# ShenhanQian/SpeechDrivesTemplates

Measured on AMD Instinct MI355X. Metric: training clips/sec (64-frame, 137-kpt) voice2pose_sdt_bp, higher is better.
Workload: dtype f32 (Conv2d forward / input gradient: each fp32 operand split exactly into three bf16 numbers, six bf16 MFMA products per fp32 product, fp32 accumulation -- products exact to 2^-23; everything else fp32 arithmetic)

## Files before the change

__graft_entry__.py:

```python
import os
import subprocess
import sys

REPO = os.path.dirname(os.path.abspath(__file__))
CSRC = os.path.join(REPO, "speechdrivestemplates_amd", "csrc")
LIBDIR = os.path.join(REPO, "speechdrivestemplates_amd", "lib")
LIB = os.path.join(LIBDIR, "libsdt_hip.so")
SOURCES = ["conv.hip", "convsk.hip", "convbf.hip", "norm.hip", "misc.hip", "l0.hip", "chain1d.hip", "render.hip", "speaker_stats.hip",
           "code_pca.hip", "code_axes.hip", "code_clusters.hip", "fgd.hip", "jpeg.hip", "gif.hip", "clip_builder.hip", "optim_guard.hip",
           "tensor_hist.hip", "reg_loss.hip", "clip_metrics.hip", "long_demo.hip"]
HIPCC = os.environ.get("HIPCC", "/opt/rocm/bin/hipcc")
FLAGS = ["--offload-arch=gfx950", "-O3", "-std=c++17", "-fPIC", "-munsafe-fp-atomics", "-Wno-unused-result", "-Wno-unused-value"]


def _stale(out, deps):
    if not os.path.exists(out):
        return True
    t = os.path.getmtime(out)
    return any(os.path.getmtime(d) > t for d in deps)


TUNING_LIB = os.path.join(LIBDIR, "libsdt_hip_tuning.so")


def _headers():
    return sorted(os.path.join(CSRC, f) for f in os.listdir(CSRC) if f.endswith(".h")) + [os.path.join(REPO, "include", "sdt_hip.h")]


def _start_compiles(prefix, extra, force):
    objs, procs = [], []
    for src in SOURCES:
        s = os.path.join(CSRC, src)
        o = os.path.join(LIBDIR, prefix + src.replace(".hip", ".o"))
        objs.append(o)
        if force or _stale(o, [s] + _headers()):
            procs.append((src, subprocess.Popen([HIPCC] + FLAGS + extra + ["-c", s, "-o", o])))
    return objs, procs


def _finish(lib, objs, procs, force):
    for src, p in procs:
        if p.wait() != 0:
            raise RuntimeError("hipcc failed on %s (%s)" % (src, os.path.basename(lib)))
    if force or procs or _stale(lib, objs):
        subprocess.check_call([HIPCC, "--offload-arch=gfx950", "-shared", "-fPIC", "-o", lib] + objs)


def build_tuning(force=False):
    os.makedirs(LIBDIR, exist_ok=True)
    objs, procs = _start_compiles("tuning_", ["-DSDT_TUNING"], force)
    _finish(TUNING_LIB, objs, procs, force)
    return TUNING_LIB


def build(force=False):
    os.makedirs(LIBDIR, exist_ok=True)
    objs, procs = _start_compiles("", [], force)
    tobjs, tprocs = _start_compiles("tuning_", ["-DSDT_TUNING"], force)
    _finish(LIB, objs, procs, force)
    _finish(TUNING_LIB, tobjs, tprocs, force)
    if REPO not in sys.path:
        sys.path.insert(0, REPO)
    import speechdrivestemplates_amd
    from speechdrivestemplates_amd import _lib
    _lib.load()


def make_pipeline(cfg_name, n_clips, batch_global=None, state=None, log_interval=10 ** 9, sys_opts=None):
    if REPO not in sys.path:
        sys.path.insert(0, REPO)
    from speechdrivestemplates_amd.config import get_cfg_defaults
    from speechdrivestemplates_amd.core.datasets import gesture_dataset as gd
    from speechdrivestemplates_amd.core.pipelines import get_pipeline
    cfg = get_cfg_defaults()
    cfg.merge_from_file(os.path.join(REPO, "configs", cfg_name + ".yaml"))
    opts = ["DATASET.NAME", "SyntheticGestureDataset", "DATASET.SYNTHETIC_CLIPS", n_clips, "SYS.LOG_INTERVAL", log_interval]
    if batch_global is not None:
        opts += ["TRAIN.BATCH_SIZE", batch_global]
    for k, v in (sys_opts or {}).items():
        opts += ["SYS." + k, v]
    cfg.merge_from_list(opts)
    cfg.freeze()
    pipe = get_pipeline(cfg.PIPELINE_TYPE)(cfg)
    pipe.num_train_samples = n_clips
    pipe.train_dataset = gd.SyntheticGestureDataset(cfg=cfg, num_clips=n_clips)
    kw = {}
    if cfg.PIPELINE_TYPE == "Voice2Pose" and cfg.VOICE2POSE.GENERATOR.CLIP_CODE.EXTERNAL_CODE:
        import numpy as np
        import torch
        kw["external_codes"] = torch.from_numpy(np.random.Generator(np.random.PCG64(9)).standard_normal(
            (n_clips, cfg.VOICE2POSE.GENERATOR.CLIP_CODE.DIMENSION)).astype("float32"))
    pipe.setup_model(cfg, state_dict=None if state is None else {"module." + k: v for k, v in state.items()}, **kw)
    pipe.setup_optimizer()
# ... 43 lines not shown
```

include/sdt_hip.h:

```cpp
#ifndef SDT_HIP_H
#define SDT_HIP_H

#include <stdint.h>

#ifdef __cplusplus
extern "C" {
#endif

#define SDT_MAX_TAPS 20

enum sdt_status { SDT_OK = 0, SDT_ERR_ARG = -1, SDT_ERR_LAUNCH = -2, SDT_ERR_UNSUPPORTED = -3 };
enum sdt_dtype { SDT_F32 = 0, SDT_BF16 = 1 };

const char* sdt_last_error(void);
int sdt_abi_version(void);

typedef struct sdt_conv_geom {
    int32_t B, Hi, Wi, Cin;
    int32_t Ho, Wo;
    int32_t Hy, Wy, Cout;
    int32_t sy, sx;
    int32_t osy, osx, ooy, oox;
    int32_t ntaps, Tw;
    int32_t dy[SDT_MAX_TAPS], dx[SDT_MAX_TAPS], wt[SDT_MAX_TAPS];
// ... 98 lines not shown
                         int64_t rows, int C, float eps, float slope, void* stream);
int sdt_colnorm_bwd_f32(const float* dz, const float* y, float* dy, double* sums, const float* mean,
                        const float* rstd, const float* gamma, const float* beta, float* dgamma,
                        float* dbeta, int G, int64_t R, int C, float slope, int stats_ready, void* stream);
int sdt_colnorm_bwd_t(const void* dz, int dz_dtype, const void* y, int y_dtype, void* dy, int dy_dtype, double* sums, const float* mean,
                      const float* rstd, const float* gamma, const float* beta, float* dgamma,
                      float* dbeta, int G, int64_t R, int C, float slope, int stats_ready, void* stream);

int sdt_l0_block_fwd_f32(const float* mel, const float* w, float* z, double* mom, float* mean, float* rstd,
                         const float* gamma, const float* beta, float* running_mean, float* running_var,
                         int64_t* num_batches_tracked, int B, int H, int W, int groups, float eps, float momentum,
                         float slope, void* stream);
int sdt_l0_block_bwd_f32(const float* dz, const float* mel, const float* w, const float* mean, const float* rstd,
                         const float* gamma, const float* beta, const double* mom, double* sums, float* dw, float* dgamma,
                         float* dbeta, int B, int H, int W, int groups, float slope, void* stream);
int sdt_l0_block_fwd_t(const float* mel, const float* w, void* z, int z_dtype, double* mom, float* mean, float* rstd,
                       const float* gamma, const float* beta, float* running_mean, float* running_var,
                       int64_t* num_batches_tracked, int B, int H, int W, int groups, float eps, float momentum,
                       float slope, void* stream);
int sdt_l0_block_bwd_t(const void* dz, int dz_dtype, const float* mel, const float* w, const float* mean, const float* rstd,
                       const float* gamma, const float* beta, const double* mom, double* sums, float* dw, float* dgamma,
                       float* dbeta, int B, int H, int W, int groups, float slope, void* stream);

int sdt_rownorm_fwd_f32(const float* y, float* z, float* mean, float* rstd, int64_t rows, int C,
                        float eps, float slope, void* stream);
int sdt_rownorm_bwd_f32(const float* dz, const float* y, const float* mean, const float* rstd, float* dy,
                        int64_t rows, int C, float slope, void* stream);
int sdt_rownorm_slabs_fwd_f32(const float* partial, int nslab, float* y, float* z, float* mean, float* rstd,
                              int64_t rows, int C, float eps, float slope, void* stream);

int sdt_resize_concat_fwd_f32(const float* x, const float* table, const int64_t* idx, float* out,
                              int B, int H, int W, int C, int T, int D, void* stream);
int sdt_resize_concat_bwd_f32(const float* dout, const int64_t* idx, float* dx, float* dtable,
                              int B, int H, int W, int C, int T, int D, void* stream);

int sdt_upsample_add_fwd_f32(const float* prev, const float* skip, float* out, int B, int Ti, int To, int C, void* stream);
int sdt_upsample_add_bwd_f32(const float* dout, float* dprev, int B, int Ti, int To, int C, void* stream);

enum { SDT_CHAIN_PLAIN = 0, SDT_CHAIN_NORM = 1, SDT_CHAIN_UPADD = 2 };
typedef struct sdt_chain1d_layer {
    int32_t Ti, To, Cin, k, stride, pad;
    int32_t in_mode;
    int32_t src_a, src_b;
    int32_t reserved;
    const float* w;
    const float* wt;
    float* y;
    float* x;
    float* dy;
    float* dx;
} sdt_chain1d_layer;
int sdt_chain1d_supported(const sdt_chain1d_layer* layers, int nlayers, int B);
int sdt_chain1d_fwd_f32(const sdt_chain1d_layer* layers, int nlayers, const float* x0, float* zout, int B, float slope, float eps,
                        int math, void* counters, void* err, void* stream);
int sdt_chain1d_bwd_f32(const sdt_chain1d_layer* layers, int nlayers, const float* gz, int B, float slope, float eps, int need_dx0,
                        int math, void* counters, void* err, void* stream);

int sdt_l1_loss_fwd_f32(const float* pred, const float* gt, int64_t n, float lambda, double* partial, float* loss, void* stream);
int sdt_l1_loss_bwd_f32(const float* pred, const float* gt, const float* gout, int64_t n, float lambda, float* dpred, void* stream);
int sdt_reg_loss_fwd_f32(const float* pred, const float* gt, const float* score, const float* chan_w, int B, int T, int C,
                         double lambda_reg, double lambda_vel, float min_conf, double* partial, int64_t* counts, float* losses,
                         double* denom, void* stream);
int sdt_reg_loss_bwd_f32(const float* pred, const float* gt, const float* score, const float* chan_w, const float* gout_reg,
                         const float* gout_vel, const double* denom, int B, int T, int C, double lambda_reg, double lambda_vel,
                         float min_conf, float* dpred, void* stream);
int sdt_mse_const_fwd_f32(const float* scores, int64_t n, float target, float lambda, float* loss, void* stream);
int sdt_mse_const_bwd_f32(const float* scores, const float* gout, int64_t n, float target, float lambda, float* dscores, void* stream);

int sdt_code_kl_fwd_f32(const float* table, const int64_t* idx, int N, int B, int D, float lambda,
                        float* code_out, float* loss, int32_t* valid, void* stream);
int sdt_code_kl_bwd_f32(const float* code, const int32_t* valid, const float* gout, const int64_t* idx,
                        int N, int B, int D, float lambda, float* dtable, void* stream);

int sdt_final_metrics_f64(const float* pred, const float* gt, const double* mean, const double* std,
                          const double* scale, int hierarchical, int B, int T, int K,
                          double* final_pred, double* final_gt, double* work, double* metrics, void* stream);

int sdt_adam_step_f32(float* p, const float* g, float* m, float* v, int64_t n, const float* lr_dev, float beta1,
                      float beta2, float eps, float weight_decay, float grad_scale, void* state_dev, void* stream);

int sdt_stft_frames_f32(const float* audio, float* hops, int B, int L, int nhops, void* stream);
int sdt_mel_fb_f32(const float* spec, const float* fb, const int32_t* bin_lo, const int32_t* bin_hi, float* mel, int B, int F,
                   int nfreq, int nmel, void* stream);

int sdt_rows_scatter_add_f32(const float* src, const int64_t* idx, float* dst, int N, int B, int D, void* stream);

int sdt_time_diff_fwd_f32(const float* x, float* y, int B, int T, int C, void* stream);
int sdt_time_diff_bwd_f32(const float* dy, float* dx, int B, int T, int C, void* stream);

int sdt_clip_poses_prepare_f32(const float* raw, const int64_t* idx, const float* mean, const float* std, float* poses,
                               float* score, int N, int Tstore, int B, int T, int hierarchical, void* stream);
int sdt_rows_gather_f32(const float* src, const int64_t* idx, float* dst, int N, int B, int64_t n_cols, void* stream);

typedef struct sdt_render_instance {
    int64_t pose;
    double off_x, off_y;
    double scale;
    int32_t shift_x;
    int32_t clip_x0, clip_x1;
    int32_t reserved;
} sdt_render_instance;

int64_t sdt_render_workspace_bytes(int n_images, int n_inst, int K);
int sdt_render_edges(int K);
int sdt_render_prepare_f64(const double* poses, int64_t n_poses, int K, const sdt_render_instance* inst, int n_images, int n_inst,
                           int H, int W, void* workspace, int64_t workspace_bytes, int32_t* skipped, void* stream);
int sdt_render_skeleton_u8(const void* workspace, int64_t workspace_bytes, int n_images, int n_inst, int K, int H, int W,
                           uint8_t* out, int64_t out_bytes, void* stream);

int64_t sdt_speaker_stats_state_bytes(int num_chunks, int num_frames);
int sdt_speaker_stats_accumulate(int pass, int elem_bytes, const void* poses, int64_t poses_elems, int64_t chunk_pitch, int num_chunks,
                                 int num_frames, int window, int64_t first_row, int64_t rows_per_chunk, const double* mean137, void* state,
                                 int64_t state_bytes, void* stream);
int sdt_speaker_stats_finalize(int pass, const void* state, int64_t state_bytes, int num_chunks, int num_frames, double* out137,
                               double* out242, double* counts, int64_t* first_bad_row, int32_t* flags, void* stream);

int64_t sdt_code_pca_workspace_bytes(int64_t n_rows, int dim);
int sdt_code_pca_moments(const float* x, int64_t n_rows, int dim, void* workspace, int64_t workspace_bytes, double* mean, double* cov,
                         int64_t* first_bad_row, void* stream);
int sdt_code_pca_eigh(const double* cov, int dim, int max_sweeps, double rel_tol, double* evals, double* comps, double* info, int32_t* err,
                      void* stream);
int sdt_code_pca_project(const float* x, int64_t n_rows, int dim, const double* mean, const double* comps, double* X, void* workspace,
                         int64_t workspace_bytes, double* limits, void* stream);
int sdt_code_pca_raster(const double* X, int64_t n_rows, const double* axis_limits, const uint8_t* table, int table_len, int H, int W,
                        int margin, int marker_px, uint32_t* counts, int64_t counts_elems, uint8_t* out, int64_t out_bytes, void* stream);

int sdt_code_axes_eigh(const double* cov, int dim, int max_sweeps, double rel_tol, double* evals, double* comps, double* info, int32_t* err,
                       void* stream);
int sdt_code_axes_project(const float* x, int64_t n_rows, int dim, const double* mean, const double* comps, double* P, void* stream);
int64_t sdt_code_axes_quantiles_workspace_bytes(int64_t n_rows, int dim, int n_ranks);
int sdt_code_axes_quantiles(const double* P, int64_t n_rows, int dim, const int64_t* ranks, int n_ranks, double* out, void* workspace,
                            int64_t workspace_bytes, void* stream);
int64_t sdt_code_axes_nearest_workspace_bytes(int64_t n_rows, int dim, int64_t n_queries);
int sdt_code_axes_nearest(const float* x, int64_t n_rows, int dim, const double* queries, int64_t n_queries, int64_t* index, double* dist2,
                          int64_t* first_bad_query, void* workspace, int64_t workspace_bytes, void* stream);

int64_t sdt_code_clusters_seed_workspace_bytes(int64_t n_rows, int dim);
int sdt_code_clusters_seed_update(const float* x, int64_t n_rows, int dim, const int64_t* seeds, int j, int first, double* m, void* workspace,
                                  int64_t workspace_bytes, void* stream);
int sdt_code_clusters_seed_pick(const double* m, int64_t n_rows, int mode, double u, int64_t* seeds, int j, double* info, void* workspace,
                                int64_t workspace_bytes, void* stream);
int sdt_code_clusters_assign(const float* x, int64_t n_rows, int dim, const double* centers, int k, int32_t* labels, int first, int64_t* changed,
                             void* stream);
int64_t sdt_code_clusters_update_workspace_bytes(int64_t n_rows, int dim, int k);
int sdt_code_clusters_update(const float* x, int64_t n_rows, int dim, const int32_t* labels, int k, double* centers, int32_t* counts,
                             void* workspace, int64_t workspace_bytes, void* stream);
int64_t sdt_code_clusters_final_workspace_bytes(int64_t n_rows, int dim, int k);
int sdt_code_clusters_final(const float* x, int64_t n_rows, int dim, const double* centers, int k, int32_t* labels, double* centers_out,
                            int32_t* counts, double* within_ss, double* inertia, int64_t* code_index, double* code_dist2, int32_t* order,
                            void* workspace, int64_t workspace_bytes, void* stream);

int64_t sdt_fgd_state_bytes(int dim);
int sdt_fgd_accumulate(const float* x0, int d0, const float* x1, int d1, int64_t rows, void* state, int64_t state_bytes,
                       int64_t rows_seen_base, void* stream);
int sdt_fgd_finalize(const void* const* states_a, const void* const* states_b, int num_states, int dim, int dim_used, int max_sweeps,
                     double rel_tol, double* out, int32_t* err, void* stream);

#define SDT_JPEG_TABLE_WORDS 672
#define SDT_JPEG_ERR_STAGE 1
#define SDT_JPEG_ERR_RANGE 2
int64_t sdt_jpeg_workspace_bytes(int n, int H, int W);
int64_t sdt_jpeg_intervals(int n, int H, int W);
int sdt_jpeg_measure(const uint8_t* frames, int64_t frames_bytes, int n, int H, int W, const uint32_t* tables, void* workspace,
                     int64_t workspace_bytes, int64_t* offsets, int64_t offsets_elems, int32_t* err, void* stream);
int sdt_jpeg_pack(const void* workspace, int64_t workspace_bytes, int n, int H, int W, const uint32_t* tables, const int64_t* offsets,
                  int64_t offsets_elems, uint8_t* out, int64_t out_bytes, int32_t* err, void* stream);
// ... 71 lines not shown
```

speechdrivestemplates_amd/_lib.py:

```python
import ctypes as C
import os

_HERE = os.path.dirname(os.path.abspath(__file__))
LIB_PATH = os.environ.get("SDT_HIP_LIB") or os.path.join(_HERE, "lib", "libsdt_hip.so")
MAX_TAPS = 20
ABI_VERSION = 5


class ConvGeom(C.Structure):
    _fields_ = [(n, C.c_int32) for n in
                ("B", "Hi", "Wi", "Cin", "Ho", "Wo", "Hy", "Wy", "Cout", "sy", "sx", "osy", "osx", "ooy", "oox",
                 "ntaps", "Tw")] + [("dy", C.c_int32 * MAX_TAPS), ("dx", C.c_int32 * MAX_TAPS), ("wt", C.c_int32 * MAX_TAPS)]


class NormBwd(C.Structure):
    _fields_ = [("y", C.c_void_p), ("mean", C.c_void_p), ("rstd", C.c_void_p), ("gamma", C.c_void_p), ("beta", C.c_void_p),
                ("sums", C.c_void_p), ("slope", C.c_float), ("groups", C.c_int32)]


class WtDesc(C.Structure):
    _fields_ = [("w", C.c_void_p), ("wt", C.c_void_p), ("w16", C.c_void_p), ("wt16", C.c_void_p), ("cout", C.c_int32), ("taps", C.c_int32),
                ("cin", C.c_int32), ("tile_begin", C.c_int32), ("planes", C.c_int32), ("reserved", C.c_int32)]


class ChainLayer(C.Structure):
    _fields_ = [("Ti", C.c_int32), ("To", C.c_int32), ("Cin", C.c_int32), ("k", C.c_int32), ("stride", C.c_int32), ("pad", C.c_int32),
                ("in_mode", C.c_int32), ("src_a", C.c_int32), ("src_b", C.c_int32), ("reserved", C.c_int32),
                ("w", C.c_void_p), ("wt", C.c_void_p), ("y", C.c_void_p), ("x", C.c_void_p), ("dy", C.c_void_p), ("dx", C.c_void_p)]


CHAIN_PLAIN, CHAIN_NORM, CHAIN_UPADD = 0, 1, 2
_p, _i, _i64, _f = C.c_void_p, C.c_int, C.c_int64, C.c_float
_G = C.POINTER(ConvGeom)

SIGNATURES = {
    "sdt_conv_taps_f32": [_p, _p, _p, _p, _G, _p],
    "sdt_conv_dw_f32": [_p, _p, _p, _G, _p],
    "sdt_conv_dw_det_f32": [_p, _p, _p, _G, _p, _i64, _p],
    "sdt_conv_taps_splitk_hint": [_G],
    "sdt_conv_taps_splitk_f32": [_p, _p, _p, _p, _G, _i, _p, _p],
    "sdt_splitk_reduce_f32": [_p, _p, _p, _i64, _i, _i, _p],
    "sdt_conv_taps_variant": [_G],
    "sdt_conv1d_small_used": [_G, _i, _i],
    "sdt_conv_dw_variant": [_G],
    "sdt_weight_transpose_f32": [_p, _p, _i, _i, _i, _p],
    "sdt_weight_transpose_batched_f32": [_p, _i, _i, _p],
    "sdt_set_conv_math": [_i],
    "sdt_col_sum_f32": [_p, _p, _i64, _i, _p],
    "sdt_colnorm_fwd_f32": [_p, _p, _p, _p, _p, _p, _p, _p, _p, _p, _i, _i64, _i, _f, _f, _f, _i, _p],
    "sdt_colnorm_fwd_t": [_p, _i, _p, _i, _p, _p, _p, _p, _p, _p, _p, _p, _i, _i64, _i, _f, _f, _f, _i, _p],
    "sdt_conv_taps_stats_supported": [_G, _i],
    "sdt_conv_taps_stats_f32": [_p, _p, _p, _p, _G, _p, _i, _p],
    "sdt_colnorm_eval_f32": [_p, _p, _p, _p, _p, _p, _i64, _i, _f, _f, _p],
    "sdt_colnorm_bwd_f32": [_p, _p, _p, _p, _p, _p, _p, _p, _p, _p, _i, _i64, _i, _f, _i, _p],
    "sdt_colnorm_bwd_t": [_p, _i, _p, _i, _p, _i, _p, _p, _p, _p, _p, _p, _p, _i, _i64, _i, _f, _i, _p],
    "sdt_conv_taps_multi_f32": [_p, _p, _p, _G, _i, _i, _p, C.POINTER(NormBwd), _p],
    "sdt_l0_block_fwd_f32": [_p, _p, _p, _p, _p, _p, _p, _p, _p, _p, _p, _i, _i, _i, _i, _f, _f, _f, _p],
    "sdt_l0_block_bwd_f32": [_p, _p, _p, _p, _p, _p, _p, _p, _p, _p, _p, _p, _i, _i, _i, _i, _f, _p],
    "sdt_l0_block_fwd_t": [_p, _p, _p, _i, _p, _p, _p, _p, _p, _p, _p, _p, _i, _i, _i, _i, _f, _f, _f, _p],
    "sdt_l0_block_bwd_t": [_p, _i, _p, _p, _p, _p, _p, _p, _p, _p, _p, _p, _p, _i, _i, _i, _i, _f, _p],
    "sdt_rownorm_fwd_f32": [_p, _p, _p, _p, _i64, _i, _f, _f, _p],
    "sdt_rownorm_bwd_f32": [_p, _p, _p, _p, _p, _i64, _i, _f, _p],
    "sdt_rownorm_slabs_fwd_f32": [_p, _i, _p, _p, _p, _p, _i64, _i, _f, _f, _p],
    "sdt_resize_concat_fwd_f32": [_p, _p, _p, _p, _i, _i, _i, _i, _i, _i, _p],
    "sdt_resize_concat_bwd_f32": [_p, _p, _p, _p, _i, _i, _i, _i, _i, _i, _p],
    "sdt_upsample_add_fwd_f32": [_p, _p, _p, _i, _i, _i, _i, _p],
    "sdt_conv_dw_group_plan": [C.POINTER(_G), _i, _p, C.POINTER(C.c_int64)],
    "sdt_conv_dw_group_f32": [C.POINTER(C.c_void_p), C.POINTER(C.c_void_p), C.POINTER(C.c_void_p), _i, _p, _p, _p, _p],
    "sdt_chain1d_supported": [C.POINTER(ChainLayer), _i, _i],
    "sdt_chain1d_fwd_f32": [C.POINTER(ChainLayer), _i, _p, _p, _i, _f, _f, _i, _p, _p, _p],
    "sdt_chain1d_bwd_f32": [C.POINTER(ChainLayer), _i, _p, _i, _f, _f, _i, _i, _p, _p, _p],
    "sdt_upsample_add_bwd_f32": [_p, _p, _i, _i, _i, _i, _p],
    "sdt_l1_loss_fwd_f32": [_p, _p, _i64, _f, _p, _p, _p],
    "sdt_l1_loss_bwd_f32": [_p, _p, _p, _i64, _f, _p, _p],
    "sdt_reg_loss_fwd_f32": [_p, _p, _p, _p, _i, _i, _i, C.c_double, C.c_double, _f, _p, _p, _p, _p, _p],
    "sdt_reg_loss_bwd_f32": [_p, _p, _p, _p, _p, _p, _p, _i, _i, _i, C.c_double, C.c_double, _f, _p, _p],
    "sdt_mse_const_fwd_f32": [_p, _i64, _f, _f, _p, _p],
    "sdt_mse_const_bwd_f32": [_p, _p, _i64, _f, _f, _p, _p],
    "sdt_code_kl_fwd_f32": [_p, _p, _i, _i, _i, _f, _p, _p, _p, _p],
    "sdt_code_kl_bwd_f32": [_p, _p, _p, _p, _i, _i, _i, _f, _p, _p],
    "sdt_final_metrics_f64": [_p, _p, _p, _p, _p, _i, _i, _i, _i, _p, _p, _p, _p, _p],
    "sdt_adam_step_f32": [_p, _p, _p, _p, _i64, _p, _f, _f, _f, _f, _f, _p, _p],
    "sdt_stft_frames_f32": [_p, _p, _i, _i, _i, _p],
    "sdt_mel_fb_f32": [_p, _p, _p, _p, _p, _i, _i, _i, _i, _p],
    "sdt_rows_scatter_add_f32": [_p, _p, _p, _i, _i, _i, _p],
    "sdt_time_diff_fwd_f32": [_p, _p, _i, _i, _i, _p],
    "sdt_time_diff_bwd_f32": [_p, _p, _i, _i, _i, _p],
    "sdt_clip_poses_prepare_f32": [_p, _p, _p, _p, _p, _p, _i, _i, _i, _i, _i, _p],
    "sdt_rows_gather_f32": [_p, _p, _p, _i, _i, _i64, _p],
    "sdt_convsk_supported": [_G, _i],
    "sdt_convsk_grid": [],
    "sdt_convsk_set_wg_per_cu": [_i],
    "sdt_convsk_set_f32_split": [_i],
    "sdt_convsk_set_reserved_slots": [_i],
    "sdt_convsk_plan_build": [_G, _i, _i, _i, _p, _i64],
    "sdt_convsk_dw_supported": [_G],
    "sdt_convsk_dw_plan_build": [_G, _p, _i64],
    "sdt_convsk_dw_f32": [_p, _p, _p, _p, _p, _p, _i64, _i64, _p],
    "sdt_convsk_f32": [_p, _p, _p, _p, _p, _p, _p, C.c_uint, _p, C.POINTER(NormBwd), _i64, _i64, _i64, _p],
    "sdt_convsk_bf16": [_p, _p, _p, _p, _p, _p, _p, C.c_uint, _p, C.POINTER(NormBwd), _i64, _i64, _i64, _p],
    "sdt_convsk_f32_w3": [_p, _p, _p, _p, _p, _p, _p, C.c_uint, _p, C.POINTER(NormBwd), _i64, _i64, _i64, _p],
    "sdt_convsk_supported_t": [_G, _i, _i],
    "sdt_convsk_plan_build_t": [_G, _i, _i, _i, _i, _i, _p, _i64],
    "sdt_convsk_dw_supported_t": [_G, _i],
    "sdt_convsk_dw_plan_build_t": [_G, _i, _p, _i64],
    "sdt_convsk_dw_bf16": [_p, _p, _p, _p, _p, _p, _i64, _i64, _p],
    "sdt_convsk_set_spin_limit": [C.c_uint],
    "sdt_convsk_set_k_order": [_i],
    "sdt_convsk_set_dw_wide_tiles": [_i],
    "sdt_render_workspace_bytes": [_i, _i, _i],
    "sdt_render_edges": [_i],
    "sdt_render_prepare_f64": [_p, _i64, _i, _p, _i, _i, _i, _i, _p, _i64, _p, _p],
    "sdt_render_skeleton_u8": [_p, _i64, _i, _i, _i, _i, _i, _p, _i64, _p],
    "sdt_speaker_stats_state_bytes": [_i, _i],
    "sdt_speaker_stats_accumulate": [_i, _i, _p, _i64, _i64, _i, _i, _i, _i64, _i64, _p, _p, _i64, _p],
    "sdt_speaker_stats_finalize": [_i, _p, _i64, _i, _i, _p, _p, _p, _p, _p, _p],
    "sdt_code_pca_workspace_bytes": [_i64, _i],
    "sdt_code_pca_moments": [_p, _i64, _i, _p, _i64, _p, _p, _p, _p],
    "sdt_code_pca_eigh": [_p, _i, _i, C.c_double, _p, _p, _p, _p, _p],
    "sdt_code_pca_project": [_p, _i64, _i, _p, _p, _p, _p, _i64, _p, _p],
    "sdt_code_pca_raster": [_p, _i64, _p, _p, _i, _i, _i, _i, _i, _p, _i64, _p, _i64, _p],
    "sdt_code_axes_eigh": [_p, _i, _i, C.c_double, _p, _p, _p, _p, _p],
    "sdt_code_axes_project": [_p, _i64, _i, _p, _p, _p, _p],
    "sdt_code_axes_quantiles_workspace_bytes": [_i64, _i, _i],
    "sdt_code_axes_quantiles": [_p, _i64, _i, _p, _i, _p, _p, _i64, _p],
    "sdt_code_axes_nearest_workspace_bytes": [_i64, _i, _i64],
    "sdt_code_axes_nearest": [_p, _i64, _i, _p, _i64, _p, _p, _p, _p, _i64, _p],
    "sdt_code_clusters_seed_workspace_bytes": [_i64, _i],
    "sdt_code_clusters_seed_update": [_p, _i64, _i, _p, _i, _i, _p, _p, _i64, _p],
    "sdt_code_clusters_seed_pick": [_p, _i64, _i, C.c_double, _p, _i, _p, _p, _i64, _p],
    "sdt_code_clusters_assign": [_p, _i64, _i, _p, _i, _p, _i, _p, _p],
    "sdt_code_clusters_update_workspace_bytes": [_i64, _i, _i],
    "sdt_code_clusters_update": [_p, _i64, _i, _p, _i, _p, _p, _p, _i64, _p],
    "sdt_code_clusters_final_workspace_bytes": [_i64, _i, _i],
    "sdt_code_clusters_final": [_p, _i64, _i, _p, _i, _p, _p, _p, _p, _p, _p, _p, _p, _p, _i64, _p],
    "sdt_fgd_state_bytes": [_i],
    "sdt_fgd_accumulate": [_p, _i, _p, _i, _i64, _p, _i64, _i64, _p],
    "sdt_fgd_finalize": [C.POINTER(C.c_void_p), C.POINTER(C.c_void_p), _i, _i, _i, _i, C.c_double, _p, _p, _p],
    "sdt_jpeg_workspace_bytes": [_i, _i, _i],
    "sdt_jpeg_intervals": [_i, _i, _i],
    "sdt_jpeg_measure": [_p, _i64, _i, _i, _i, _p, _p, _i64, _p, _i64, _p, _p],
    "sdt_jpeg_pack": [_p, _i64, _i, _i, _i, _p, _p, _i64, _p, _i64, _p, _p],
    "sdt_gif_workspace_bytes": [_i, _i, _i],
    "sdt_gif_quantise": [_p, _i64, _i, _i, _i, _i, _i, _p, _i64, _p, _i64, _p, _p, _i64, _p],
    "sdt_gif_measure": [_p, _i64, _i, _i, _i, _p, _i64, _p, _i64, _p, _p],
    "sdt_gif_pack": [_p, _i64, _i, _i, _i, _p, _i64, _p, _i64, _p, _p],
    "sdt_clip_workspace_bytes": [_i64],
    "sdt_clip_frame_flags": [_i, _p, _p, _i64, _p, _p, _p, _p],
    "sdt_clip_scan": [_p, _p, _i64, _p, _p, _p],
    "sdt_clip_shoulder_means": [_p, _p, _i64, _i, _p, _p],
    "sdt_clip_window_candidates": [_i64, _i, _i, _i],
    "sdt_clip_windows": [_p, _i64, _i, _i, _i, _p, _i64, _p, _i64, _p, _p],
    "sdt_clip_gather_poses": [_i, _p, _i64, _p, _i64, _i, C.c_double, _i, _p, _i64, _p],
    "sdt_clip_pcm_to_mono_f32": [_i, _p, _i64, _i, _i64, _p, _i64, _p],
    "sdt_clip_resample_lds_bytes": [_i, _i, _i],
    "sdt_clip_resample_f32": [_p, _i64, _p, _i, _i, _i, _i64, _p, _i64, _p],
    "sdt_clip_gather_audio": [_p, _i64, _p, _p, _i64, _i64, _p, _i64, _p, _p],
    "sdt_grad_sumsq_partials": [],
    "sdt_optim_guard_pass_elems": [_i],
    "sdt_grad_sumsq_f64": [_p, _i64, _p, _p],
    "sdt_optim_guard_prep": [C.POINTER(C.c_void_p), _i, _f, C.c_double, _i, _p, _p],
    "sdt_adam_step_guarded_f32": [_p, _p, _p, _p, _i64, _p, _f, _f, _f, _f, _p, _p, _f, _p, _p],
    "sdt_tensor_hist_threads": [],
    "sdt_tensor_hist_chunk": [],
    "sdt_tensor_hist_buckets": [],
    "sdt_tensor_hist_max_segments": [],
    "sdt_tensor_hist_plan": [_p, _i, _i64, _p, _p, _i64, _p],
# ... 99 lines not shown
```

speechdrivestemplates_amd/mel.py:

```python
import math

import torch
from torch import nn

from . import ops


def htk_filterbank(n_freqs, f_min, f_max, n_mels, sample_rate):
    freqs = torch.linspace(0, sample_rate // 2, n_freqs)
    mel_lo = 2595.0 * math.log10(1.0 + f_min / 700.0)
    mel_hi = 2595.0 * math.log10(1.0 + f_max / 700.0)
    edges = 700.0 * (10 ** (torch.linspace(mel_lo, mel_hi, n_mels + 2) / 2595.0) - 1.0)
    width = edges[1:] - edges[:-1]
    dist = edges.unsqueeze(0) - freqs.unsqueeze(1)
    rising = -dist[:, :-2] / width[:-1]
    falling = dist[:, 2:] / width[1:]
    return torch.minimum(rising, falling).clamp_min(0.0)


class _Window(nn.Module):
    def __init__(self, win_length):
        super().__init__()
        self.register_buffer('window', torch.hann_window(win_length, periodic=True))


class _MelScale(nn.Module):
    def __init__(self, n_freqs, f_min, f_max, n_mels, sample_rate):
        super().__init__()
        self.register_buffer('fb', htk_filterbank(n_freqs, f_min, f_max, n_mels, sample_rate))


class MelSpectrogram(nn.Module):
    def __init__(self, sample_rate=16000, n_fft=512, win_length=400, hop_length=160, f_min=55, f_max=7500.0, n_mels=80):
        super().__init__()
        if (n_fft, win_length, hop_length) != (ops.N_FFT, ops.WIN, ops.HOP):
            raise NotImplementedError('the STFT kernel path is specialised to n_fft=512 / win=400 / hop=160')
        self.spectrogram = _Window(win_length)
        self.mel_scale = _MelScale(n_fft // 2 + 1, float(f_min), float(f_max), n_mels, sample_rate)
        self._basis = None
        self._basis_key = None
        self._bins = None
        self._bins_key = None

    def _dft_basis(self):
        w = self.spectrogram.window
        key = (w.data_ptr(), w._version, w.device)
        if self._basis is None or self._basis_key != key:
            self._basis = ops.dft_basis(w).to(w.device)
            self._basis_key = key
        return self._basis

    def _fb_bins(self):
        fb = self.mel_scale.fb
        key = (fb.data_ptr(), fb._version, fb.device)
        if self._bins is None or self._bins_key != key:
            self._bins = ops.fb_bin_ranges(fb)
            self._bins_key = key
        return self._bins

    @torch.no_grad()
    def forward(self, waveform):
        return ops.mel_spectrogram(waveform, self._dft_basis(), self.mel_scale.fb, self._fb_bins())
```

speechdrivestemplates_amd/ops.py:

```python
import functools
import math
import os

import torch

from . import _lib
from ._lib import ConvGeom, check

LEAKY_SLOPE = 0.2
BN_EPS, BN_MOMENTUM = 1e-5, 0.1


def out_size(n, k, s, p):
    return (n + 2 * p - k) // s + 1


def _geom(**kw):
    g = ConvGeom()
    taps = kw.pop("taps")
    for k, v in kw.items():
        setattr(g, k, int(v))
    g.ntaps = len(taps)
    assert 0 < g.ntaps <= _lib.MAX_TAPS, "kernel has too many taps (%d)" % g.ntaps
    for i, (dy, dx, wt) in enumerate(taps):
# ... 1668 lines not shown
class TimeDiffFn(torch.autograd.Function):

    @staticmethod
    def forward(ctx, x):
        _req_cuda(x)
        x = x.contiguous()
        B, T, C = x.shape
        y = torch.empty((B, T - 1, C), device=x.device, dtype=torch.float32)
        check(_lib.load().sdt_time_diff_fwd_f32(_p(x), _p(y), B, T, C, _stream()))
        ctx.dims = (B, T, C)
        return y

    @staticmethod
    def backward(ctx, g):
        B, T, C = ctx.dims
        g = g.contiguous()
        dx = torch.empty((B, T, C), device=g.device, dtype=torch.float32)
        check(_lib.load().sdt_time_diff_bwd_f32(_p(g), _p(dx), B, T, C, _stream()))
        return dx


def clip_poses_prepare(raw_store, idx, mean, std, num_frames, hierarchical):
    _req_cuda(raw_store, idx, mean, std)
    assert raw_store.dim() == 4 and raw_store.shape[2:] == (3, 137) and raw_store.is_contiguous() and raw_store.dtype == torch.float32
    assert idx.dtype == torch.int64 and mean.numel() == 242 and std.numel() == 242
    N, Tstore = raw_store.shape[:2]
    B = idx.numel()
    poses = torch.empty((B, num_frames, 2, 121), device=raw_store.device, dtype=torch.float32)
    score = torch.empty_like(poses)
    idx, mean, std = idx.contiguous(), mean.contiguous(), std.contiguous()
    check(_lib.load().sdt_clip_poses_prepare_f32(_p(raw_store), _p(idx), _p(mean), _p(std),
                                                 _p(poses), _p(score), N, Tstore, B, num_frames, int(bool(hierarchical)), _stream()))
    return poses, score


def rows_gather(src, idx):
    _req_cuda(src, idx)
    assert src.dim() == 2 and src.is_contiguous() and src.dtype == torch.float32 and idx.dtype == torch.int64
    dst = torch.empty((idx.numel(), src.shape[1]), device=src.device, dtype=torch.float32)
    idx = idx.contiguous()
    check(_lib.load().sdt_rows_gather_f32(_p(src), _p(idx), _p(dst), src.shape[0], idx.numel(), src.shape[1], _stream()))
    return dst


def final_metrics(pred, gt, mean, std, scale, hierarchical, want_final=True):
    _req_cuda(pred, gt, mean, std, scale)
    B, T, _, K = pred.shape
    pred, gt = pred.contiguous(), gt.contiguous()
    dev = pred.device
    fp = torch.empty((B, T, 2, K), device=dev, dtype=torch.float64) if want_final else None
    fg = torch.empty((B, T, 2, K), device=dev, dtype=torch.float64) if want_final else None
    work = _ARENA.take(3 * B * T + 4, dev)
    metrics = torch.empty(2, device=dev, dtype=torch.float64)
    mean, std, scale = mean.contiguous(), std.contiguous(), scale.contiguous()
    check(_lib.load().sdt_final_metrics_f64(_p(pred), _p(gt), _p(mean), _p(std), _p(scale),
                                            1 if hierarchical else 0, B, T, K, _p(fp), _p(fg), _p(work), _p(metrics), _stream()))
    return fp, fg, metrics


N_FFT, WIN, HOP, N_FREQ = 512, 400, 160, 257


def dft_basis(window):
    w = window.detach().double().cpu()
    k = torch.arange(WIN, dtype=torch.float64)
    f = torch.arange(N_FREQ, dtype=torch.float64)
    ang = 2.0 * math.pi * torch.outer(f, k + (N_FFT - WIN) // 2) / N_FFT
    basis = torch.zeros(2 * N_FREQ, 3 * HOP, dtype=torch.float64)
    basis[0::2, :WIN] = torch.cos(ang) * w
    basis[1::2, :WIN] = -torch.sin(ang) * w
    return basis.float().reshape(2 * N_FREQ, 3, HOP).contiguous()


def fb_bin_ranges(fb):
    nz = (fb.detach().cpu() != 0)
    n_freq = nz.shape[0]
    idx = torch.arange(n_freq).unsqueeze(1)
    lo = torch.where(nz, idx, torch.full_like(idx, n_freq)).min(0).values
    hi = torch.where(nz, idx + 1, torch.zeros_like(idx)).max(0).values
    lo = torch.minimum(lo, hi)
    return lo.to(torch.int32).to(fb.device), hi.to(torch.int32).to(fb.device)


def mel_spectrogram(audio, basis, fb, bins=None):
    _req_cuda(audio, basis, fb)
    lo, hi = bins if bins is not None else fb_bin_ranges(fb)
    lib = _lib.load()
    audio = audio.contiguous()
    B, L = audio.shape
    F = 1 + L // HOP
    nh = F + 2
    st = _stream()
    hops = torch.empty((B, nh, HOP), device=audio.device, dtype=torch.float32)
    check(lib.sdt_stft_frames_f32(_p(audio), _p(hops), B, L, nh, st))
    g = _geom(B=B, Hi=1, Wi=nh, Cin=HOP, Ho=1, Wo=F, Hy=1, Wy=F, Cout=2 * N_FREQ, sy=1, sx=1, osy=1, osx=1, ooy=0, oox=0,
              Tw=3, taps=[(0, 0, 0), (0, 1, 1), (0, 2, 2)])
    spec = torch.empty((B, F, 2 * N_FREQ), device=audio.device, dtype=torch.float32)
    math = _CONV_MATH_NOW[0]
    if math != 0:
        check(lib.sdt_set_conv_math(0))
    try:
        check(lib.sdt_conv_taps_f32(_p(hops), _p(basis), None, _p(spec), g, st))
    finally:
        if math != 0:
            check(lib.sdt_set_conv_math(math))
    nmel = fb.shape[1]
    mel = torch.empty((B, nmel, F), device=audio.device, dtype=torch.float32)
    fb = fb.contiguous()
    check(lib.sdt_mel_fb_f32(_p(spec), _p(fb), _p(lo), _p(hi), _p(mel), B, F, N_FREQ, nmel, st))
    return mel


def adam_step(p, g, m, v, lr_dev, state_dev, beta1=0.9, beta2=0.999, eps=1e-8, weight_decay=0.0, grad_scale=1.0):
    _req_cuda(p, g, m, v, lr_dev, state_dev)
    check(_lib.load().sdt_adam_step_f32(_p(p), _p(g), _p(m), _p(v), p.numel(), _p(lr_dev), beta1, beta2, eps, weight_decay,
                                        grad_scale, _p(state_dev), _stream()))


GUARD_WORDS = 4


def grad_sumsq_partials():
    return int(_lib.load().sdt_grad_sumsq_partials())


def optim_guard_pass_elems(which):
    return int(_lib.load().sdt_optim_guard_pass_elems({'sumsq': 0, 'adam': 1}[which]))


def grad_sumsq(g, partial):
    _req_cuda(g, partial)
    if g.dtype != torch.float32 or partial.dtype != torch.float64 or partial.numel() < grad_sumsq_partials():
        raise ValueError('grad_sumsq: g must be fp32 and partial %d float64 elements' % grad_sumsq_partials())
    check(_lib.load().sdt_grad_sumsq_f64(_p(g), g.numel(), _p(partial), _stream()))
    return partial


def optim_guard_prep(partials, guard, grad_scale=1.0, max_norm=0.0, skip_nonfinite=False):
    _req_cuda(guard, *partials)
    if not 1 <= len(partials) <= 4:
        raise ValueError('a step group has 1 to 4 buffers, got %d' % len(partials))
    if guard.dtype != torch.int64 or guard.numel() < GUARD_WORDS:
        raise ValueError('the guard record is %d int64 words' % GUARD_WORDS)
    import ctypes as C
    arr = (C.c_void_p * len(partials))(*[_p(t) for t in partials])
    check(_lib.load().sdt_optim_guard_prep(arr, len(partials), grad_scale, float(max_norm), int(bool(skip_nonfinite)), _p(guard), _stream()))


def adam_step_guarded(p, g, m, v, lr_dev, state_dev, guard, beta1=0.9, beta2=0.999, eps=1e-8, weight_decay=0.0, ema=None, ema_decay=0.0):
    _req_cuda(p, g, m, v, lr_dev, state_dev, guard)
    if ema is not None:
        _req_cuda(ema)
        if ema.numel() != p.numel() or ema.dtype != torch.float32:
            raise ValueError('the EMA buffer must match the parameter buffer')
    check(_lib.load().sdt_adam_step_guarded_f32(_p(p), _p(g), _p(m), _p(v), p.numel(), _p(lr_dev), beta1, beta2, eps, weight_decay,
                                                _p(guard), _p(ema), ema_decay, _p(state_dev), _stream()))


def _check_sizes(status):
    if status == -3:
        raise ValueError('libsdt_hip: %s' % _lib.load().sdt_last_error().decode())
    check(status)


def tensor_hist_constants():
    lib = _lib.load()
    return {k: int(getattr(lib, 'sdt_tensor_hist_' + k)()) for k in ('threads', 'chunk', 'buckets', 'max_segments')}


def tensor_hist_plan(offsets, sizes, n):
    import ctypes as C
    lib = _lib.load()
    S = len(offsets)
    if len(sizes) != S:
        raise ValueError('tensor_hist_plan: %d offsets but %d sizes' % (S, len(sizes)))
    segs = torch.tensor([[int(o), int(s)] for o, s in zip(offsets, sizes)], dtype=torch.int64).reshape(S, 2)
    n_chunks = C.c_int64(0)
    _check_sizes(lib.sdt_tensor_hist_plan(_p(segs) if S else None, S, int(n), None, None, 0, C.addressof(n_chunks)))
    seg_plan = torch.zeros((S, 3), dtype=torch.int64)
    chunk_plan = torch.zeros((max(1, n_chunks.value), 2), dtype=torch.int64)
    _check_sizes(lib.sdt_tensor_hist_plan(_p(segs), S, int(n), _p(seg_plan), _p(chunk_plan), n_chunks.value, C.addressof(n_chunks)))
    return seg_plan, chunk_plan[:n_chunks.value]


def tensor_hist(flat, seg_plan, chunk_plan, edges, scale, counts, tallies, stats, partials):
    _req_cuda(flat, seg_plan, chunk_plan, edges, counts, tallies, stats, partials)
    S, nc = seg_plan.shape[0], chunk_plan.shape[0]
    if flat.dtype != torch.float32 or not flat.is_contiguous():
        raise ValueError('tensor_hist: flat must be a contiguous fp32 buffer')
    if counts.dtype != torch.int64 or tallies.dtype != torch.int64 or stats.dtype != torch.float64 or edges.dtype != torch.float64 \
            or counts.numel() < S * (edges.numel() - 1) or tallies.numel() < 3 * S or stats.numel() < 4 * S or partials.numel() < 4 * nc \
# ... 5 lines not shown
```

Before: 5696.

## Fuse STFT power into compact-bin MFMA kernel for mel spectrogram

Adds a dedicated STFT kernel that computes only the frequency bins the mel filterbank actually uses, over a compacted, zero-trimmed DFT basis, and squares real/imag inside the kernel to emit power directly. A new filterbank kernel then reads that compact power tensor. This replaces the generic full-spectrum conv plus separate filterbank pass, cutting wasted MACs on dead bins and the full complex spectrum round trip. The compacted basis is cached per module, and it adds code paths that must match the old numerics.

```diff
diff --git a/__graft_entry__.py b/__graft_entry__.py
--- a/__graft_entry__.py
+++ b/__graft_entry__.py
@@ -8,7 +8,7 @@
 LIB = os.path.join(LIBDIR, "libsdt_hip.so")
 SOURCES = ["conv.hip", "convsk.hip", "convbf.hip", "norm.hip", "misc.hip", "l0.hip", "chain1d.hip", "render.hip", "speaker_stats.hip",
            "code_pca.hip", "code_axes.hip", "code_clusters.hip", "fgd.hip", "jpeg.hip", "gif.hip", "clip_builder.hip", "optim_guard.hip",
-           "tensor_hist.hip", "reg_loss.hip", "clip_metrics.hip", "long_demo.hip"]
+           "tensor_hist.hip", "reg_loss.hip", "clip_metrics.hip", "long_demo.hip", "mel.hip"]
 HIPCC = os.environ.get("HIPCC", "/opt/rocm/bin/hipcc")
 FLAGS = ["--offload-arch=gfx950", "-O3", "-std=c++17", "-fPIC", "-munsafe-fp-atomics", "-Wno-unused-result", "-Wno-unused-value"]
 
diff --git a/include/sdt_hip.h b/include/sdt_hip.h
--- a/include/sdt_hip.h
+++ b/include/sdt_hip.h
@@ -204,6 +204,12 @@
 int sdt_stft_frames_f32(const float* audio, float* hops, int B, int L, int nhops, void* stream);
 int sdt_mel_fb_f32(const float* spec, const float* fb, const int32_t* bin_lo, const int32_t* bin_hi, float* mel, int B, int F,
                    int nfreq, int nmel, void* stream);
+int sdt_mel_compact_map(int k0, int k1, int32_t* src_row, int cap);
+int sdt_mel_basis_compact_f32(const float* basis, int nfreq, int k0, int k1, float* out, void* stream);
+int sdt_stft_power_f32(const float* hops, const float* basis_c, float* power, int B, int nhops, int F, int nbins_live, int ncols,
+                       int klen, void* stream);
+int sdt_mel_fb_power_f32(const float* power, const float* fb, const int32_t* bin_lo, const int32_t* bin_hi, float* mel, int B, int F,
+                         int k0, int nbins_live, int nmel, void* stream);
 
 int sdt_rows_scatter_add_f32(const float* src, const int64_t* idx, float* dst, int N, int B, int D, void* stream);
 
diff --git a/speechdrivestemplates_amd/_lib.py b/speechdrivestemplates_amd/_lib.py
--- a/speechdrivestemplates_amd/_lib.py
+++ b/speechdrivestemplates_amd/_lib.py
@@ -83,6 +83,10 @@
     "sdt_adam_step_f32": [_p, _p, _p, _p, _i64, _p, _f, _f, _f, _f, _f, _p, _p],
     "sdt_stft_frames_f32": [_p, _p, _i, _i, _i, _p],
     "sdt_mel_fb_f32": [_p, _p, _p, _p, _p, _i, _i, _i, _i, _p],
+    "sdt_mel_compact_map": [_i, _i, _p, _i],
+    "sdt_mel_basis_compact_f32": [_p, _i, _i, _i, _p, _p],
+    "sdt_stft_power_f32": [_p, _p, _p, _i, _i, _i, _i, _i, _i, _p],
+    "sdt_mel_fb_power_f32": [_p, _p, _p, _p, _p, _i, _i, _i, _i, _i, _p],
     "sdt_rows_scatter_add_f32": [_p, _p, _p, _i, _i, _i, _p],
     "sdt_time_diff_fwd_f32": [_p, _p, _i, _i, _i, _p],
     "sdt_time_diff_bwd_f32": [_p, _p, _i, _i, _i, _p],
diff --git a/speechdrivestemplates_amd/csrc/mel.hip b/speechdrivestemplates_amd/csrc/mel.hip
--- /dev/null
+++ b/speechdrivestemplates_amd/csrc/mel.hip
@@ -0,0 +1,216 @@
+#include "common.h"
+
+#define STP_BM 64
+#define STP_BINS 32
+#define STP_BK 32
+#define STP_LDP 36
+#define STP_K 480
+#define STP_OOB 0x80000000u
+
+__host__ __device__ static inline int mel_compact_src(int n, int k0, int k1) {
+    const int bin = k0 + (n / (2 * STP_BINS)) * STP_BINS + (n % STP_BINS);
+    return bin < k1 ? 2 * bin + ((n / STP_BINS) & 1) : -1;
+}
+static inline int mel_compact_cols(int k0, int k1) { return cdiv(k1 - k0, STP_BINS) * 2 * STP_BINS; }
+
+__global__ __launch_bounds__(256) void mel_basis_compact_kernel(const float* __restrict__ basis, float* __restrict__ out, int k0, int k1,
+                                                                int ncols) {
+    const int total = ncols * STP_K;
+    for (int i = blockIdx.x * 256 + threadIdx.x; i < total; i += gridDim.x * 256) {
+        const int n = i / STP_K, k = i - n * STP_K;
+        const int src = mel_compact_src(n, k0, k1);
+        out[i] = src >= 0 ? basis[(size_t)src * STP_K + k] : 0.f;
+    }
+}
+
+__global__ __launch_bounds__(128) void stft_power_kernel(const float* __restrict__ X, const float* __restrict__ W, float* __restrict__ P,
+                                                         const int B, const int nh, const int F, const int nbl, const int ncols,
+                                                         const int nsteps) {
+    __shared__ __attribute__((aligned(16))) float sA[STP_BM * STP_LDP];
+    __shared__ __attribute__((aligned(16))) float sB[2 * STP_BINS * STP_LDP];
+    const int tid = threadIdx.x, lane = tid & 63, wave = tid >> 6;
+    const int M = B * F;
+    const int nmb = (M + STP_BM - 1) / STP_BM, nnb = ncols / (2 * STP_BINS);
+    const int lin = xcd_remap(blockIdx.x, nmb * nnb);
+    const int m0 = (lin / nnb) * STP_BM, nt = lin % nnb;
+
+    const int kv = tid & 7, r0 = tid >> 3;
+    const __amdgpu_buffer_rsrc_t rsX = __builtin_amdgcn_make_buffer_rsrc((void*)X, 0, (int)((unsigned)B * nh * 160u * 4u), 0x00020000);
+    const __amdgpu_buffer_rsrc_t rsW = __builtin_amdgcn_make_buffer_rsrc((void*)W, 0, (int)((unsigned)ncols * STP_K * 4u), 0x00020000);
+    unsigned aoff[4], boff[4];
+#pragma unroll
+    for (int i = 0; i < 4; ++i) {
+        const int m = m0 + r0 + 16 * i;
+        if (m < M) {
+            const int b = m / F, f = m - b * F;
+            aoff[i] = (unsigned)((b * nh + f) * 160 + kv * 4) * 4u;
+        } else {
+            aoff[i] = STP_OOB;
+        }
+        boff[i] = (unsigned)((nt * 2 * STP_BINS + r0 + 16 * i) * STP_K + kv * 4) * 4u;
+    }
+    f32x4 ra[4], rb[4];
+    auto load = [&](int step) {
+        const int cs = step * STP_BK * 4;
+#pragma unroll
+        for (int i = 0; i < 4; ++i) ra[i] = __builtin_bit_cast(f32x4, __builtin_amdgcn_raw_buffer_load_b128(rsX, (int)aoff[i], cs, 0));
+#pragma unroll
+        for (int i = 0; i < 4; ++i) rb[i] = __builtin_bit_cast(f32x4, __builtin_amdgcn_raw_buffer_load_b128(rsW, (int)boff[i], cs, 0));
+    };
+
+    f32x16 are, aim;
+#pragma unroll
+    for (int r = 0; r < 16; ++r) are[r] = aim[r] = 0.f;
+    const float* pa = sA + (wave * 32 + (lane & 31)) * STP_LDP + (lane >> 5) * 4;
+    const float* pb = sB + (lane & 31) * STP_LDP + (lane >> 5) * 4;
+
+    load(0);
+    for (int step = 0; step < nsteps; ++step) {
+#pragma unroll
+        for (int i = 0; i < 4; ++i) *(f32x4*)&sA[(r0 + 16 * i) * STP_LDP + kv * 4] = ra[i];
+#pragma unroll
+        for (int i = 0; i < 4; ++i) *(f32x4*)&sB[(r0 + 16 * i) * STP_LDP + kv * 4] = rb[i];
+        __syncthreads();
+        if (step + 1 < nsteps) load(step + 1);
+#pragma unroll
+        for (int j = 0; j < 4; ++j) {
+            const f32x4 a = *(const f32x4*)(pa + j * 8);
+            const f32x4 br = *(const f32x4*)(pb + j * 8);
+            const f32x4 bi = *(const f32x4*)(pb + STP_BINS * STP_LDP + j * 8);
+#pragma unroll
+            for (int e = 0; e < 4; ++e) {
+                are = __builtin_amdgcn_mfma_f32_32x32x2f32(a[e], br[e], are, 0, 0, 0);
+                aim = __builtin_amdgcn_mfma_f32_32x32x2f32(a[e], bi[e], aim, 0, 0, 0);
+            }
+        }
+        __syncthreads();
+    }
+
+    const int bin = nt * STP_BINS + (lane & 31);
+    if (bin < nbl) {
+#pragma unroll
+        for (int r = 0; r < 16; ++r) {
+            const int m = m0 + wave * 32 + (r & 3) + 8 * (r >> 2) + 4 * (lane >> 5);
+            if (m < M) P[(size_t)m * nbl + bin] = __fadd_rn(__fmul_rn(are[r], are[r]), __fmul_rn(aim[r], aim[r]));
+        }
+    }
+}
+
+#define MELP_FT 16
+template <int MAXF>
+__global__ __launch_bounds__(320) void mel_fb_power_kernel(const float* __restrict__ P, const float* __restrict__ fb,
+                                                           const int* __restrict__ bin_lo, const int* __restrict__ bin_hi,
+                                                           float* __restrict__ mel, int M, int F, int nmel, int nbl, int k0) {
+    extern __shared__ float smem[];
+    const int ldp = nbl + 1;
+    float* sP = smem;
+    float* sO = smem + MELP_FT * ldp;
+    const int row0 = blockIdx.x * MELP_FT;
+    const int nrows = min(MELP_FT, M - row0);
+    const int total = nrows * nbl;
+    const float* src = P + (size_t)row0 * nbl;
+    for (int e = threadIdx.x * 4; e < MELP_FT * nbl; e += 320 * 4) {
+        float v[4] = {0.f, 0.f, 0.f, 0.f};
+        if (e + 3 < total) {
+            const f32x4 q = *(const f32x4*)(src + e);
+            v[0] = q[0], v[1] = q[1], v[2] = q[2], v[3] = q[3];
+        } else {
+#pragma unroll
+            for (int c = 0; c < 4; ++c)
+                if (e + c < total) v[c] = src[e + c];
+        }
+        int r = e / nbl, k = e - r * nbl;
+#pragma unroll
+        for (int c = 0; c < 4; ++c) {
+            if (r < MELP_FT) sP[r * ldp + k] = v[c];
+            if (++k == nbl) k = 0, ++r;
+        }
+    }
+    __syncthreads();
+    const int npg = 320 / nmel;
+    const int m = threadIdx.x % nmel, fg = threadIdx.x / nmel;
+    if (fg < npg) {
+        float acc[MAXF];
+#pragma unroll
+        for (int i = 0; i < MAXF; ++i) acc[i] = 0.f;
+        const int ka = max(bin_lo[m], k0), kb = min(bin_hi[m], k0 + nbl);
+        for (int k = ka; k < kb; ++k) {
+            const float w = fb[(size_t)k * nmel + m];
+#pragma unroll
+            for (int i = 0; i < MAXF; ++i) {
+                const int fr = fg + npg * i;
+                if (fr < MELP_FT) acc[i] = fmaf(w, sP[fr * ldp + k - k0], acc[i]);
+            }
+        }
+#pragma unroll
+        for (int i = 0; i < MAXF; ++i) {
+            const int fr = fg + npg * i;
+            if (fr < MELP_FT) sO[m * (MELP_FT + 1) + fr] = acc[i];
+        }
+    }
+    __syncthreads();
+    for (int o = threadIdx.x; o < nmel * MELP_FT; o += 320) {
+        const int mm = o / MELP_FT, fr = o - mm * MELP_FT;
+        const int row = row0 + fr;
+        if (row < M) {
+            const int b = row / F, f = row - b * F;
+            mel[((size_t)b * nmel + mm) * F + f] = sO[mm * (MELP_FT + 1) + fr];
+        }
+    }
+}
+
+extern "C" int sdt_mel_compact_map(int k0, int k1, int32_t* src_row, int cap) {
+    SDT_CHECK_ARG(k0 >= 0 && k1 > k0 && k1 <= 32768, "bad bin range");
+    const int ncols = mel_compact_cols(k0, k1);
+    if (src_row != nullptr) {
+        SDT_CHECK_ARG(cap >= ncols, "map buffer too small");
+        for (int n = 0; n < ncols; ++n) src_row[n] = mel_compact_src(n, k0, k1);
+    }
+    return ncols;
+}
+
+extern "C" int sdt_mel_basis_compact_f32(const float* basis, int nfreq, int k0, int k1, float* out, void* stream) {
+    SDT_CHECK_ARG(basis && out && nfreq > 0 && nfreq <= 32768 && k0 >= 0 && k1 > k0 && k1 <= nfreq, "bad argument");
+    const int ncols = mel_compact_cols(k0, k1);
+    hipLaunchKernelGGL(mel_basis_compact_kernel, dim3(std::min(cdiv(ncols * STP_K, 256), 1024)), dim3(256), 0, (hipStream_t)stream, basis, out,
+                       k0, k1, ncols);
+    SDT_LAUNCH_CHECK();
+    return SDT_OK;
+}
+
+extern "C" int sdt_stft_power_f32(const float* hops, const float* basis_c, float* power, int B, int nhops, int F, int nbins_live, int ncols,
+                                  int klen, void* stream) {
+    SDT_CHECK_ARG(hops && basis_c && power && B > 0 && F > 0 && nhops >= F + 2, "bad argument (a frame spans 3 hops: nhops >= F + 2)");
+    SDT_CHECK_ARG(nbins_live > 0 && ncols == mel_compact_cols(0, nbins_live), "ncols does not match the live bin count");
+    SDT_CHECK_ARG(klen > 0 && klen <= STP_K, "klen must be in (0, 480]");
+    SDT_CHECK_ARG((((uintptr_t)hops | (uintptr_t)basis_c) % 16) == 0, "buffers must be 16-byte aligned");
+    SDT_CHECK_ARG((int64_t)B * nhops * 160 * 4 < (int64_t)0x7fff0000 && (int64_t)ncols * STP_K * 4 < (int64_t)0x7fff0000 &&
+                      (int64_t)B * F < (int64_t)0x7fff0000 / 64,
+                  "tensor too large for 32-bit buffer offsets");
+    const int64_t tiles = cdiv64((int64_t)B * F, STP_BM) * (ncols / (2 * STP_BINS));
+    SDT_CHECK_ARG(tiles < (int64_t)0x7fffffff, "too many tiles");
+    hipLaunchKernelGGL(stft_power_kernel, dim3((unsigned)tiles), dim3(128), 0, (hipStream_t)stream, hops, basis_c, power, B, nhops, F, nbins_live,
+                       ncols, cdiv(klen, STP_BK));
+    SDT_LAUNCH_CHECK();
+    return SDT_OK;
+}
+
+extern "C" int sdt_mel_fb_power_f32(const float* power, const float* fb, const int32_t* bin_lo, const int32_t* bin_hi, float* mel, int B,
+                                    int F, int k0, int nbins_live, int nmel, void* stream) {
+    SDT_CHECK_ARG(power && fb && bin_lo && bin_hi && mel && B > 0 && F > 0 && k0 >= 0 && nbins_live > 0, "bad argument");
+    SDT_CHECK_ARG(nmel > 0 && nmel <= 320, "unsupported mel count");
+    SDT_CHECK_ARG(((uintptr_t)power % 16) == 0, "power must be 16-byte aligned");
+    SDT_CHECK_ARG((int64_t)B * F < (int64_t)0x7fffffff - MELP_FT, "too many frames");
+    const size_t lds = ((size_t)MELP_FT * (nbins_live + 1) + (size_t)nmel * (MELP_FT + 1)) * sizeof(float);
+    SDT_CHECK_ARG(lds <= 64 * 1024, "too many frequency bins");
+    const int M = B * F;
+    const int per_thread = cdiv(MELP_FT, std::min(320 / nmel, MELP_FT));
+#define SDT_MELP(N) hipLaunchKernelGGL(mel_fb_power_kernel<N>, dim3(cdiv(M, MELP_FT)), dim3(320), lds, (hipStream_t)stream, power, fb, bin_lo, \
+                                       bin_hi, mel, M, F, nmel, nbins_live, k0)
+    if (per_thread <= 4) SDT_MELP(4);
+    else if (per_thread <= 8) SDT_MELP(8);
+    else SDT_MELP(16);
+#undef SDT_MELP
+    SDT_LAUNCH_CHECK();
+    return SDT_OK;
+}
diff --git a/speechdrivestemplates_amd/mel.py b/speechdrivestemplates_amd/mel.py
--- a/speechdrivestemplates_amd/mel.py
+++ b/speechdrivestemplates_amd/mel.py
@@ -41,6 +41,8 @@
         self._basis_key = None
         self._bins = None
         self._bins_key = None
+        self._compact = None
+        self._compact_key = None
 
     def _dft_basis(self):
         w = self.spectrogram.window
@@ -58,6 +60,15 @@
             self._bins_key = key
         return self._bins
 
+    def _compact_basis(self):
+        basis, bins = self._dft_basis(), self._fb_bins()
+        key = (self._basis_key, self._bins_key)
+        if self._compact_key != key:
+            self._compact = ops.mel_basis_compact(basis, bins)
+            self._compact_key = key
+        return self._compact
+
     @torch.no_grad()
     def forward(self, waveform):
-        return ops.mel_spectrogram(waveform, self._dft_basis(), self.mel_scale.fb, self._fb_bins())
+        compact = self._compact_basis() if ops.MEL_FUSED else None
+        return ops.mel_spectrogram(waveform, self._dft_basis(), self.mel_scale.fb, self._fb_bins(), compact)
diff --git a/speechdrivestemplates_amd/ops.py b/speechdrivestemplates_amd/ops.py
--- a/speechdrivestemplates_amd/ops.py
+++ b/speechdrivestemplates_amd/ops.py
@@ -1774,9 +1774,51 @@
     return lo.to(torch.int32).to(fb.device), hi.to(torch.int32).to(fb.device)
 
 
-def mel_spectrogram(audio, basis, fb, bins=None):
+MEL_FUSED = True
+
+
+def fb_live_range(bins):
+    lo, hi = bins[0].cpu(), bins[1].cpu()
+    live = hi > lo
+    if not bool(live.any()):
+        return 0, 0
+    return int(lo[live].min()), int(hi[live].max())
+
+
+def _mel_compact_cols(k0, k1, ptr=None, cap=0):
+    n = _lib.load().sdt_mel_compact_map(k0, k1, ptr, cap)
+    if n < 0:
+        check(n)
+    return n
+
+
+def mel_compact_map(k0, k1):
+    ncols = _mel_compact_cols(k0, k1)
+    src = torch.empty(ncols, dtype=torch.int32)
+    _mel_compact_cols(k0, k1, src.data_ptr(), ncols)
+    return src
+
+
+def mel_basis_compact(basis, bins):
+    _req_cuda(basis)
+    k0, k1 = fb_live_range(bins)
+    if k1 <= k0:
+        return None
+    lib = _lib.load()
+    ncols = _mel_compact_cols(k0, k1)
+    basis = basis.contiguous()
+    out = torch.empty((ncols, 3, HOP), device=basis.device, dtype=torch.float32)
+    check(lib.sdt_mel_basis_compact_f32(_p(basis), basis.shape[0] // 2, k0, k1, _p(out), _stream()))
+    used = (out.reshape(ncols, 3 * HOP) != 0).any(0).nonzero()
+    klen = int(used.max()) + 1 if used.numel() else 1
+    return out, k0, k1, klen
+
+
+def mel_spectrogram(audio, basis, fb, bins=None, compact=None):
     _req_cuda(audio, basis, fb)
-    lo, hi = bins if bins is not None else fb_bin_ranges(fb)
+    if bins is None:
+        bins, compact = fb_bin_ranges(fb), None
+    lo, hi = bins
     lib = _lib.load()
     audio = audio.contiguous()
     B, L = audio.shape
@@ -1785,6 +1827,17 @@
     st = _stream()
     hops = torch.empty((B, nh, HOP), device=audio.device, dtype=torch.float32)
     check(lib.sdt_stft_frames_f32(_p(audio), _p(hops), B, L, nh, st))
+    nmel = fb.shape[1]
+    mel = torch.empty((B, nmel, F), device=audio.device, dtype=torch.float32)
+    fb = fb.contiguous()
+    if MEL_FUSED and compact is None:
+        compact = mel_basis_compact(basis, bins)
+    if MEL_FUSED and compact is not None:
+        basis_c, k0, k1, klen = compact
+        power = torch.empty((B, F, k1 - k0), device=audio.device, dtype=torch.float32)
+        check(lib.sdt_stft_power_f32(_p(hops), _p(basis_c), _p(power), B, nh, F, k1 - k0, basis_c.shape[0], klen, st))
+        check(lib.sdt_mel_fb_power_f32(_p(power), _p(fb), _p(lo), _p(hi), _p(mel), B, F, k0, k1 - k0, nmel, st))
+        return mel
     g = _geom(B=B, Hi=1, Wi=nh, Cin=HOP, Ho=1, Wo=F, Hy=1, Wy=F, Cout=2 * N_FREQ, sy=1, sx=1, osy=1, osx=1, ooy=0, oox=0,
               Tw=3, taps=[(0, 0, 0), (0, 1, 1), (0, 2, 2)])
     spec = torch.empty((B, F, 2 * N_FREQ), device=audio.device, dtype=torch.float32)
@@ -1796,9 +1849,6 @@
     finally:
         if math != 0:
             check(lib.sdt_set_conv_math(math))
-    nmel = fb.shape[1]
-    mel = torch.empty((B, nmel, F), device=audio.device, dtype=torch.float32)
-    fb = fb.contiguous()
     check(lib.sdt_mel_fb_f32(_p(spec), _p(fb), _p(lo), _p(hi), _p(mel), B, F, N_FREQ, nmel, st))
     return mel
 
```

Result: no change. 5714 (median of 6 runs) (+0.3%).
